# mousecpn/Boosting-R-CNN

Measured on AMD Instinct MI355X. Metric: images/sec (1333x800) Boosting R-CNN R50-PAFPN inference, higher is better.
Workload: dtype f32; 1 GPU; boosting_rcnn_r50_pafpn_1x_utdac.py inference (model(return_loss=False, rescale=True): device pass + result copy + bbox2result), batch 8 x 3x800x1344 per GPU, f32 MFMA conv stack, 1000 pre-NMS / 256 proposals per image, seeded synthetic weights; global_batch=8, parallelism=dp1

## Files before the change

### boosting-r-cnn_amd/csrc/nms.hip

```cpp
#include <cstdlib>
#include "common.h"
#include <cstring>
#include <rocprim/rocprim.hpp>

namespace {

__global__ void iota_kernel(int32_t* __restrict__ v, int32_t* __restrict__ v2, int64_t n) {
    int64_t i = (int64_t)blockIdx.x * blockDim.x + threadIdx.x;
    if (i < n) { v[i] = (int32_t)i; v2[i] = (int32_t)i; }
}

__global__ void gather_boxes_kernel(const float* __restrict__ boxes,
                                    const int32_t* __restrict__ sorted_idx,
                                    float* __restrict__ sboxes, float* __restrict__ sareas,
                                    int64_t n, int offset) {
    int64_t i = (int64_t)blockIdx.x * blockDim.x + threadIdx.x;
    if (i >= n) return;
    const float4 b = *reinterpret_cast<const float4*>(boxes + (size_t)sorted_idx[i] * 4);
    *reinterpret_cast<float4*>(sboxes + (size_t)i * 4) = b;
    sareas[i] = (b.z - b.x + offset) * (b.w - b.y + offset);
}

__global__ __launch_bounds__(64) void nms_mask_kernel(const float* __restrict__ sboxes,
                                                      const float* __restrict__ sareas,
                                                      const int32_t* __restrict__ seg_begin,
                                                      const int32_t* __restrict__ seg_end,
                                                      unsigned long long* __restrict__ mask,
                                                      int words, float thr, int offset) {
    const int col_t = blockIdx.x, row_t = blockIdx.y, seg = blockIdx.z;
    if (col_t < row_t) return;
    const int beg = seg_begin[seg], len = seg_end[seg] - beg;
    if (row_t * 64 >= len || col_t * 64 >= len) return;
    __shared__ float4 cb[64];
    __shared__ float ca[64];
    const int lane = threadIdx.x;
    const int cj = col_t * 64 + lane;
    if (cj < len) {
        cb[lane] = *reinterpret_cast<const float4*>(sboxes + (size_t)(beg + cj) * 4);
        ca[lane] = sareas[beg + cj];
    }
    __syncthreads();
    const int ri = row_t * 64 + lane;
    if (ri >= len) return;
    const float4 a = *reinterpret_cast<const float4*>(sboxes + (size_t)(beg + ri) * 4);
    const float aarea = sareas[beg + ri];
    const int ncol = min(64, len - col_t * 64);
    unsigned long long bits = 0ull;
    const int jstart = (row_t == col_t) ? lane + 1 : 0;
    for (int j = jstart; j < ncol; j++) {
        const float4 b = cb[j];
        const float xx1 = fmaxf(a.x, b.x), yy1 = fmaxf(a.y, b.y);
        const float xx2 = fminf(a.z, b.z), yy2 = fminf(a.w, b.w);
        const float w = fmaxf(0.f, xx2 - xx1 + offset), h = fmaxf(0.f, yy2 - yy1 + offset);
        const float inter = w * h;
        const float ovr = inter / (aarea + ca[j] - inter);
        if (ovr > thr) bits |= 1ull << j;
    }
    mask[(size_t)(beg + ri) * words + col_t] = bits;
}

__global__ __launch_bounds__(256) void nms_reduce_kernel(const unsigned long long* __restrict__ mask,
                                                         const int32_t* __restrict__ sorted_idx,
                                                         const int32_t* __restrict__ seg_begin,
                                                         const int32_t* __restrict__ seg_end,
                                                         int64_t* __restrict__ keep,
                                                         int32_t* __restrict__ num_keep, int words,
                                                         int max_keep) {
    extern __shared__ unsigned long long remv[];
    __shared__ int sh_count;
    const int seg = blockIdx.x, tid = threadIdx.x, lane = tid & 63, wave = tid >> 6;
    const int beg = seg_begin[seg], len = seg_end[seg] - beg;
    const int nchunk = (len + 63) >> 6;
    unsigned long long* kept_sh = remv + words;
    for (int w = tid; w < nchunk; w += 256) remv[w] = 0ull;
    if (tid == 0) sh_count = 0;
    __syncthreads();
    int count = 0;
    unsigned long long diag_next = 0ull, diag_cur = 0ull;
    if (wave == 0 && lane < len) diag_next = mask[(size_t)(beg + lane) * words];
    {
        unsigned nlo, nhi;
        asm volatile("v_mov_b32 %0, %2\n\tv_mov_b32 %1, %3"
                     : "=v"(nlo), "=v"(nhi)
                     : "v"((unsigned)diag_next), "v"((unsigned)(diag_next >> 32)));
        diag_cur = ((unsigned long long)nhi << 32) | nlo;
    }
    for (int c = 0; c < nchunk; c++) {
        const unsigned long long* mchunk = mask + (size_t)(beg + c * 64) * words;
        const int w0 = c + 1 + lane;
        unsigned long long pre[16];
#pragma unroll
        for (int j = 0; j < 16; j++) {
            const int r = wave * 16 + j;
            pre[j] = (w0 < nchunk && c * 64 + r < len) ? mchunk[(size_t)r * words + w0] : 0ull;
// ... 211 lines not shown
    if (k < num[b]) {
        const long long src = keep[(size_t)b * T + k];
        const float4 bx = *reinterpret_cast<const float4*>(c_boxes + src * 4);
        d[0] = bx.x; d[1] = bx.y; d[2] = bx.z; d[3] = bx.w; d[4] = c_scores[src];
        ids_kept[i] = c_ids[src];
    } else {
        d[0] = d[1] = d[2] = d[3] = d[4] = 0.f;
        ids_kept[i] = -1;
    }
}


__device__ __forceinline__ unsigned order_key(float f) {
    const unsigned u = __float_as_uint(f);
    return (u & 0x80000000u) ? ~u : (u | 0x80000000u);
}

template <int THREADS>
__global__ __launch_bounds__(THREADS) void seg_sort_gather_kernel(const float* __restrict__ boxes,
                                                              const float* __restrict__ scores,
                                                              const int32_t* __restrict__ seg_begin,
                                                              const int32_t* __restrict__ seg_end,
                                                              int32_t* __restrict__ idx_out, float* __restrict__ sboxes,
                                                              float* __restrict__ sareas, int offset) {
    extern __shared__ unsigned long long comp[];
    const int seg = blockIdx.x, tid = threadIdx.x;
    const int beg = seg_begin[seg], len = seg_end[seg] - beg;
    if (len <= 0) return;
    int P = 64;
    while (P < len) P <<= 1;
    for (int i = tid; i < P; i += THREADS)
        comp[i] = i < len ? (((unsigned long long)(~order_key(scores[beg + i])) << 32) | (unsigned)i) : ~0ull;
    __syncthreads();
    for (int k = 2; k <= P; k <<= 1) {
        for (int j = k >> 1; j > 0; j >>= 1) {
            for (int t = tid; t < (P >> 1); t += THREADS) {
                const int lo = ((t & ~(j - 1)) << 1) | (t & (j - 1));
                const int hi = lo | j;
                const unsigned long long a = comp[lo], b = comp[hi];
                const bool up = (lo & k) == 0;
                if ((a > b) == up) { comp[lo] = b; comp[hi] = a; }
            }
            __syncthreads();
        }
    }
    for (int i = tid; i < len; i += THREADS) {
        const int src = beg + (int)(comp[i] & 0xffffffffu);
        idx_out[beg + i] = src;
        const float4 b = *reinterpret_cast<const float4*>(boxes + (size_t)src * 4);
        *reinterpret_cast<float4*>(sboxes + (size_t)(beg + i) * 4) = b;
        sareas[beg + i] = (b.z - b.x + offset) * (b.w - b.y + offset);
    }
}

__global__ __launch_bounds__(1024) void nms_collect_sorted_kernel(const long long* __restrict__ keep,
                                                                 const int* __restrict__ num, const int* __restrict__ ranges,
                                                                 const float* __restrict__ c_boxes,
                                                                 const float* __restrict__ c_scores,
                                                                 const long long* __restrict__ c_ids,
                                                                 const float* __restrict__ new_scores,
                                                                 float* __restrict__ dets, long long* __restrict__ ids_kept,
                                                                 int* __restrict__ n_kept, int T, int L, int K) {
    extern __shared__ unsigned long long comp[];
    __shared__ int s_off[BRCNN_MAX_LEVELS + 1];
    const int b = blockIdx.x, tid = threadIdx.x;
    if (tid == 0) {
        int o = 0;
        for (int l = 0; l < L; l++) { s_off[l] = o; o += num[b * L + l]; }
        s_off[L] = o;
    }
    __syncthreads();
    const int cnt = s_off[L];
    int P = 64;
    while (P < cnt) P <<= 1;
    for (int l = 0; l < L; l++) {
        const int beg = ranges[2 * (b * L + l)], n_l = s_off[l + 1] - s_off[l];
        for (int i = tid; i < n_l; i += 1024) {
            const long long src = keep[beg + i];
            const float sc = new_scores ? new_scores[(size_t)(beg + i) * 5 + 4] : c_scores[src];
            comp[s_off[l] + i] = ((unsigned long long)(~order_key(sc)) << 32) | (unsigned)(src - (long long)b * T);
        }
    }
    for (int i = cnt + tid; i < P; i += 1024) comp[i] = ~0ull;
    __syncthreads();
    for (int k = 2; k <= P; k <<= 1) {
        for (int j = k >> 1; j > 0; j >>= 1) {
            for (int t = tid; t < (P >> 1); t += 1024) {
                const int lo = ((t & ~(j - 1)) << 1) | (t & (j - 1));
                const int hi = lo | j;
                const unsigned long long a = comp[lo], c = comp[hi];
                const bool up = (lo & k) == 0;
                if ((a > c) == up) { comp[lo] = c; comp[hi] = a; }
            }
            __syncthreads();
        }
    }
    const int kept = cnt < K ? cnt : K;
    if (tid == 0) n_kept[b] = kept;
    for (int k = tid; k < K; k += 1024) {
        float* d = dets + ((size_t)b * K + k) * 5;
        if (k < kept) {
            const unsigned long long c = comp[k];
            const size_t src = (size_t)b * T + (unsigned)(c & 0xffffffffu);
            const float4 bx = *reinterpret_cast<const float4*>(c_boxes + src * 4);
            const unsigned key = ~(unsigned)(c >> 32);
            const unsigned u = (key & 0x80000000u) ? (key & 0x7fffffffu) : ~key;
            d[0] = bx.x; d[1] = bx.y; d[2] = bx.z; d[3] = bx.w; d[4] = __uint_as_float(u);
            if (ids_kept) ids_kept[(size_t)b * K + k] = c_ids[src];
        } else {
            d[0] = d[1] = d[2] = d[3] = d[4] = 0.f;
            if (ids_kept) ids_kept[(size_t)b * K + k] = -1;
        }
    }
}

}

static int g_nms_lds_sort = getenv("BRCNN_NMS_RADIX") ? 0 : 1;

BRCNN_API size_t brcnn_nms_workspace_bytes(int64_t n, int num_segments, int64_t max_segment_len) {
    if (n <= 0 || num_segments <= 0) return 256;
    if (max_segment_len <= 0 || max_segment_len > n) max_segment_len = n;
    const int words = (int)((max_segment_len + 63) / 64);
    return carve(nullptr, n, num_segments, words).total;
}

BRCNN_API int brcnn_nms(const float* boxes, const float* scores, const int32_t* seg_begin,
                        const int32_t* seg_end, int num_segments, int64_t n, int64_t max_segment_len, float iou_threshold,
                        int offset, int max_keep, int64_t* keep, int32_t* num_keep, void* workspace,
                        size_t workspace_bytes, void* stream) {
    if (n < 0 || num_segments <= 0 || (offset != 0 && offset != 1) || !seg_begin || !seg_end || !num_keep)
        return BRCNN_EINVAL;
    hipStream_t s = (hipStream_t)stream;
    if (n == 0) {
        BRCNN_HIP_CHECK(hipMemsetAsync(num_keep, 0, sizeof(int32_t) * num_segments, s));
        return 0;
    }
    if (!boxes || !scores || !keep || !workspace || max_segment_len <= 0 || max_segment_len > n)
        return BRCNN_EINVAL;
    if (n > 0x7fffffffLL) return BRCNN_EINVAL;
    const int words = (int)((max_segment_len + 63) / 64);
    NmsWs w = carve(workspace, n, num_segments, words);
    if (w.total > workspace_bytes) return BRCNN_EINVAL;

    if (max_segment_len <= 16384 && g_nms_lds_sort) {
        int P = 64;
        while (P < max_segment_len) P <<= 1;
        static bool attr_done = false;
        if (!attr_done) {
            BRCNN_HIP_CHECK(hipFuncSetAttribute((const void*)seg_sort_gather_kernel<1024>,
                                                hipFuncAttributeMaxDynamicSharedMemorySize, 16384 * 8));
            attr_done = true;
        }
        if (max_segment_len <= 512)
            hipLaunchKernelGGL(seg_sort_gather_kernel<256>, dim3(num_segments), dim3(256), (size_t)P * 8, s, boxes, scores,
                               seg_begin, seg_end, w.idx_out, w.sboxes, w.sareas, offset);
        else
            hipLaunchKernelGGL(seg_sort_gather_kernel<1024>, dim3(num_segments), dim3(1024), (size_t)P * 8, s, boxes, scores,
                               seg_begin, seg_end, w.idx_out, w.sboxes, w.sareas, offset);
        BRCNN_LAUNCH_CHECK();
    } else {
        hipLaunchKernelGGL(iota_kernel, dim3(brcnn_cdiv(n, 256)), dim3(256), 0, s, w.idx_in, w.idx_out, n);
        BRCNN_LAUNCH_CHECK();
        size_t tmp = w.sort_tmp_bytes;
        BRCNN_HIP_CHECK((rocprim::segmented_radix_sort_pairs_desc(
            w.sort_tmp, tmp, scores, w.keys_out, (const int32_t*)w.idx_in, w.idx_out, (unsigned)n,
            (unsigned)num_segments, seg_begin, seg_end, 0, 32, s, false)));
        hipLaunchKernelGGL(gather_boxes_kernel, dim3(brcnn_cdiv(n, 256)), dim3(256), 0, s, boxes,
                           (const int32_t*)w.idx_out, w.sboxes, w.sareas, n, offset);
        BRCNN_LAUNCH_CHECK();
    }
    hipLaunchKernelGGL(nms_mask_kernel, dim3(words, words, num_segments), dim3(64), 0, s,
                       (const float*)w.sboxes, (const float*)w.sareas, seg_begin, seg_end, w.mask, words,
                       iou_threshold, offset);
    BRCNN_LAUNCH_CHECK();
    hipLaunchKernelGGL(nms_reduce_kernel, dim3(num_segments), dim3(256), (size_t)(words + 1) * 8, s,
                       (const unsigned long long*)w.mask, (const int32_t*)w.idx_out, seg_begin, seg_end,
                       keep, num_keep, words, max_keep);
    BRCNN_LAUNCH_CHECK();
    return 0;
}

BRCNN_API int brcnn_nms_prepare(const float* boxes, const float* scores, const int64_t* ids, const uint8_t* valid,
                                float* c_boxes, float* c_scores, int64_t* c_ids, float* nms_boxes, int32_t* ranges,
                                int batch, int slot, void* stream) {
    if (!boxes || !scores || !ids || !valid || !c_boxes || !c_scores || !c_ids || !nms_boxes || !ranges ||
        batch <= 0 || slot <= 0 || (long long)batch * slot >= 0x7fffffffLL)
        return BRCNN_EINVAL;
    LevelBounds lb;
    lb.num = 0;
    hipLaunchKernelGGL(nms_prepare_kernel, dim3(batch), dim3(1024), 0, (hipStream_t)stream, boxes, scores,
                       (const long long*)ids, valid, c_boxes, c_scores, (long long*)c_ids, nms_boxes, ranges, slot, lb);
    BRCNN_LAUNCH_CHECK();
    return 0;
}

BRCNN_API int brcnn_nms_prepare_levels(const float* boxes, const float* scores, const int64_t* ids, const uint8_t* valid,
                                       float* c_boxes, float* c_scores, int64_t* c_ids, float* nms_boxes,
                                       int32_t* ranges, int batch, int slot, int num_levels,
                                       const int* level_sizes_host, void* stream) {
    if (!boxes || !scores || !ids || !valid || !c_boxes || !c_scores || !c_ids || !nms_boxes || !ranges ||
        batch <= 0 || slot <= 0 || (long long)batch * slot >= 0x7fffffffLL || num_levels <= 0 ||
        num_levels > BRCNN_MAX_LEVELS || !level_sizes_host)
// ... 13 lines not shown
    BRCNN_LAUNCH_CHECK();
    return 0;
}

BRCNN_API int brcnn_nms_collect_sorted(const int64_t* keep, const int32_t* num, const int32_t* ranges,
                                       const float* c_boxes, const float* c_scores, const int64_t* c_ids,
                                       const float* new_scores5, float* dets, int64_t* ids_kept, int32_t* n_kept,
                                       int batch, int slot, int num_levels, int max_keep, void* stream) {
    if (!keep || !num || !ranges || !c_boxes || !c_scores || !c_ids || !dets || !n_kept || batch <= 0 || slot <= 0 ||
        slot > 16384 || num_levels <= 0 || num_levels > BRCNN_MAX_LEVELS || max_keep <= 0 || max_keep > slot)
        return BRCNN_EINVAL;
    int P = 64;
    while (P < slot) P <<= 1;
    static bool attr_done = false;
    if (!attr_done) {
        BRCNN_HIP_CHECK(hipFuncSetAttribute((const void*)nms_collect_sorted_kernel,
                                            hipFuncAttributeMaxDynamicSharedMemorySize, 16384 * 8));
        attr_done = true;
    }
    hipLaunchKernelGGL(nms_collect_sorted_kernel, dim3(batch), dim3(1024), (size_t)P * 8, (hipStream_t)stream,
                       (const long long*)keep, num, ranges, c_boxes, c_scores, (const long long*)c_ids, new_scores5, dets,
                       (long long*)ids_kept, n_kept, slot, num_levels, max_keep);
    BRCNN_LAUNCH_CHECK();
    return 0;
}

BRCNN_API int brcnn_nms_collect(const int64_t* keep, const int32_t* num, const float* c_boxes, const float* c_scores,
                                const int64_t* c_ids, float* dets, int64_t* ids_kept, int batch, int slot,
                                int max_keep, void* stream) {
    if (!keep || !num || !c_boxes || !c_scores || !c_ids || !dets || !ids_kept || batch <= 0 || slot <= 0 ||
        max_keep <= 0 || max_keep > slot)
        return BRCNN_EINVAL;
    const int total = batch * max_keep;
    hipLaunchKernelGGL(nms_collect_kernel, dim3((total + 255) / 256), dim3(256), 0, (hipStream_t)stream,
                       (const long long*)keep, num, c_boxes, c_scores, (const long long*)c_ids, dets,
                       (long long*)ids_kept, batch, slot, max_keep);
    BRCNN_LAUNCH_CHECK();
    return 0;
}
```

### boosting-r-cnn_amd/csrc/policy.h

```cpp
#pragma once

namespace brcnn {

struct Policy {
    int use_dma = 1;
    int force_wm = 0, force_nt = 0;
    int no_fast = 0;
    int pp_f32_n128 = 1;
    int pp_f32_mode = 1;
    int f32_tile_sk = 1;
    int f32_tile_sk_per_cu = 0;
    int f32_winograd = 1;
    int f32_winograd_chunks = 1;
    int f32_winograd_layer = 1;
    int f32_winograd_gemm = 0;
    int f32_winograd_sk = 1;
    int f32_winograd_sk_per_cu = 0;
    int f32_winograd_sk_wgs = 0;
    int f32_winograd_ring = 0;
    int f32_winograd_tower_gemm = 0;

    int dcn_fused = 1;

    int bf16_tile = 0;
// ... 4 lines not shown
    int pp128_mode = 1;
    int pp128_min_k = 4096;
    int pp128_max_t88 = 128;
    int sk_spin_limit = 1 << 24;
    int sk_drop_publish = 0;
    int stream_mode = 1;

    int wgrad_bf16_tile = 0;
    int wgrad_slabs = 1;
    int wgrad_slot_pct = 75;
    int wgrad_slot_pct_big = 75;
    int wgrad_two_pass = 24;
    int wgrad_pp_mode = 1;
    int wgrad_pp_slot_pct = 75;
    int wgrad_pp_two_pass = 24;
    int wgrad_pp_fuse = 0;

    int roi_exact = 0;
    int roi_stream_c = 3;
    int roi_prep = 0;
    int roi_rpw = 0;
    int roi_order = 1;
    int roi_gather_chunks = -1;
};
extern Policy g_policy;

struct Counters {
    int f32_tile_sk_launches = 0;
    int f32_tile_sk_wgs = 0;
    int wgrad_pp_launches = 0;
    int pp_f32_launches = 0;
    int pp_f32_rows = 0;
    int pp_f32_cols = 0;
    int pp_bf16_launches = 0;
    int pp128_bf16_launches = 0;
    int stream1x1_launches = 0;
    int sk_chain_fills = 0;
    int sk_par_fills = 0;
    int sk_last_wgs = 0;
    int bf16_tile_launches = 0;
    int bf16_tile_rows = 0;
    int bf16_tile_cols = 0;
    int bf16_tile_waves = 0;
    int bf16_tile_stages = 0;
    int wgrad_bf16_tile_launches = 0;
    int wgrad_bf16_last_tile = 0;
    int f32_winograd_launches = 0;
    int f32_winograd_tiles = 0;
    int f32_winograd_layer_launches = 0;
    int f32_winograd_layer_variant = 0;
    int f32_winograd_sk_launches = 0;
    int f32_winograd_sk_last_wgs = 0;
    int f32_winograd_tower_variant = 0;
    int f32_winograd_last_ring = 0;
    int dcn_fused_launches = 0;
    int dcn_im2col_launches = 0;
    int roi_ordered_launches = 0;
    int roi_prepared_launches = 0;
    int roi_gather_chunked = 0;
    int roi_gather_last_ch = 0;
};
extern Counters g_counters;
inline void count(int& c) { c = (c + 1) & 0x7fffffff; }

int wino_layer_rule(int tiles, int cin, int cout);
int wino_gemm_rule(int tiles, int cout);
int wino_gemm_variant(int tiles, int cout);
int wino_persistent_rule(int workgroup_tiles, int units, int cus, int per_cu);
int wino_tower_gemm_rule(int tiles, int cout);
int wino_ring_rule(int workgroup_tiles, int cin);

}
```

### boosting-r-cnn_amd/csrc/policy.hip

```cpp
#include "common.h"
#include "policy.h"

__attribute__((require_constant_initialization)) brcnn::Policy brcnn::g_policy;
__attribute__((require_constant_initialization)) brcnn::Counters brcnn::g_counters;
using brcnn::g_counters, brcnn::g_policy;

BRCNN_API int brcnn_conv_set_tile(int wm, int nt) {
    if (wm == -1) { g_policy.use_dma = nt; return 0; }
    if (wm == -3) { if (nt < 0 || nt > 2) return BRCNN_EINVAL; g_policy.pp_f32_n128 = nt; return 0; }
    if (wm == -4) { if (nt != 0 && nt != 1) return BRCNN_EINVAL; g_policy.no_fast = nt; return 0; }
    if (wm == -5) { if (nt < 0 || nt > 2) return BRCNN_EINVAL; g_policy.f32_tile_sk = nt; return 0; }
    if (wm == -7) { if (nt < 0 || nt > 8) return BRCNN_EINVAL; g_policy.f32_tile_sk_per_cu = nt; return 0; }
    if (wm == -6) return nt == 0 ? g_counters.f32_tile_sk_launches : nt == 1 ? g_counters.f32_tile_sk_wgs : BRCNN_EINVAL;
    if (wm == -9) {
        int* const c[] = {&g_counters.pp_f32_launches, &g_counters.pp_f32_rows, &g_counters.pp_f32_cols, &g_counters.pp_bf16_launches,
                          &g_counters.pp128_bf16_launches, &g_counters.stream1x1_launches, &g_counters.sk_chain_fills,
                          &g_counters.sk_par_fills, &g_counters.sk_last_wgs, &g_counters.bf16_tile_launches, &g_counters.bf16_tile_rows,
                          &g_counters.bf16_tile_cols, &g_counters.bf16_tile_waves, &g_counters.bf16_tile_stages,
                          &g_counters.wgrad_bf16_tile_launches, &g_counters.wgrad_bf16_last_tile};
        const int count = (int)(sizeof(c) / sizeof(c[0]));
        if (nt < -1 || nt >= count) return BRCNN_EINVAL;
        if (nt == -1) {
            for (int* q : c) *q = 0;
            g_counters.f32_winograd_launches = g_counters.f32_winograd_tiles = 0;
            g_counters.dcn_fused_launches = g_counters.dcn_im2col_launches = 0;
            g_counters.f32_winograd_layer_launches = g_counters.f32_winograd_layer_variant = 0;
            g_counters.f32_winograd_sk_launches = g_counters.f32_winograd_sk_last_wgs = g_counters.f32_winograd_tower_variant = 0;
            g_counters.f32_winograd_last_ring = 0;
            return 0;
        }
        const int n = *c[nt];
        *c[nt] = 0;
        return n;
    }
    if (wm == -11) {
        if (nt == 0 || nt == 1) { g_policy.f32_winograd = nt; return 0; }
        if (nt == 2) return g_policy.f32_winograd;
        if (nt >= 11 && nt <= 18) { g_policy.f32_winograd_chunks = nt - 10; return 0; }
        return BRCNN_EINVAL;
    }
    if (wm == -12) {
        if (nt != 0 && nt != 1) return BRCNN_EINVAL;
        int& c = nt == 0 ? g_counters.f32_winograd_launches : g_counters.f32_winograd_tiles;
        const int n = c;
        c = 0;
        return n;
    }
    if (wm == -13) {
        if (nt >= 0 && nt <= 2) { g_policy.dcn_fused = nt; return 0; }
        if (nt == 3) return g_policy.dcn_fused;
        if (nt != 10 && nt != 11) return BRCNN_EINVAL;
// ... 7 lines not shown
        if (nt == 3) return g_policy.f32_winograd_layer;
        if (nt >= 20 && nt <= 23) { g_policy.f32_winograd_gemm = nt - 20; return 0; }
        if (nt == 24) return g_policy.f32_winograd_gemm;
        if (nt != 10 && nt != 11) return BRCNN_EINVAL;
        int& c = nt == 10 ? g_counters.f32_winograd_layer_launches : g_counters.f32_winograd_layer_variant;
        const int n = c;
        c = 0;
        return n;
    }
    if (wm == -16) {
        if (nt >= 0 && nt <= 2) { g_policy.f32_winograd_sk = nt; return 0; }
        if (nt == 3) return g_policy.f32_winograd_sk;
        if (nt == 20 || nt == 21 || nt == 23) { g_policy.f32_winograd_tower_gemm = nt - 20; return 0; }
        if (nt == 24) return g_policy.f32_winograd_tower_gemm;
        if (nt >= 30 && nt <= 38) { g_policy.f32_winograd_sk_per_cu = nt - 30; return 0; }
        if (nt == 39) return g_policy.f32_winograd_sk_per_cu;
        if (nt == 40 || nt == 42 || nt == 43) { g_policy.f32_winograd_ring = nt - 40; return 0; }
        if (nt == 49) return g_policy.f32_winograd_ring;
        if (nt >= 1000 && nt <= 1000 + 2048) { g_policy.f32_winograd_sk_wgs = nt - 1000; return 0; }
        if (nt == 999) return g_policy.f32_winograd_sk_wgs;
        if (nt < 10 || nt > 13) return BRCNN_EINVAL;
        int& c = nt == 10 ? g_counters.f32_winograd_sk_launches : nt == 11 ? g_counters.f32_winograd_sk_last_wgs
                 : nt == 12 ? g_counters.f32_winograd_tower_variant : g_counters.f32_winograd_last_ring;
        const int n = c;
        c = 0;
        return n;
    }
    if (wm == -2) { if (nt != 0 && nt != 1 && nt != 2 && nt != 128 && nt != 256) return BRCNN_EINVAL; g_policy.pp_f32_mode = nt; return 0; }
    if ((wm != 0 && wm != 1 && wm != 2 && wm != 4) || nt < 0 || nt > 2) return BRCNN_EINVAL;
    g_policy.force_wm = wm;
    g_policy.force_nt = nt;
    return 0;
}

int brcnn::wino_gemm_rule(int tiles, int cout) {
    (void)tiles; (void)cout;
    return 3;
}

int brcnn::wino_layer_rule(int tiles, int cin, int cout) {
    if (cin != cout) return 0;
    if (cin == 256) return tiles >= 5250;
    if (cin == 512) return tiles >= 444;
    return 0;
}

// ... 136 lines not shown
```

### boosting-r-cnn_amd/dense_heads.py

```python
import copy

import torch
import torch.distributed as dist
import torch.nn as nn

from . import ops
from .blocks import (ConvModule, PackedCache, Scale, bias_init_with_prob, pack_weight, to_nhwc)
from .postprocess import batched_nms_images
from .core import (anchor_inside_flags, bbox_overlaps, const_rows, images_to_levels, multi_apply, unmap)
from .registry import (HEADS, build_anchor_generator, build_assigner, build_bbox_coder,
                       build_loss, build_sampler)

EPS = 1e-12


def cat_rows(feats):
    from .autograd import cat_rows as _cr
    return _cr(list(feats))


def _nchw_rows(lst):
    return torch.cat([t.permute(0, 2, 3, 1).reshape(-1, t.shape[1]) for t in lst], 0).float()


# ... 302 lines not shown
                for b in range(B):
                    p1, v1 = ops.rpn_decode(topk_inds[b:b + 1], reg_nhwc[lvl][b:b + 1],
                                            self._base_anchors(lvl, device), (h, w), stride,
                                            self.bbox_coder.means, self.bbox_coder.stds,
                                            img_metas[b]['img_shape'][:2], cfg.min_bbox_size,
                                            pred_scale=rs)
                    pl.append(p1)
                    vl.append(v1)
                props, valid = torch.cat(pl), torch.cat(vl)
            if cfg.min_bbox_size < 0:
                valid = torch.ones_like(valid)
            sc_l.append(score)
            pr_l.append(props)
            va_l.append(valid.bool())
            id_l.append(torch.full((B, score.shape[1]), lvl, dtype=torch.long, device=device))
        scores = torch.cat(sc_l, 1)
        props = torch.cat(pr_l, 1)
        valid = torch.cat(va_l, 1)
        ids = torch.cat(id_l, 1)
        return self._proposals_from_candidates(props, scores, ids, valid, sc_l, nms_cfg, cfg)

    @staticmethod
    def _proposals_from_candidates(props, scores, ids, valid, sc_l, nms_cfg, cfg):
        if scores.shape[1] >= nms_cfg.get('split_thr', 10000):
            from .postprocess import batched_nms_images_by_level
            return batched_nms_images_by_level(props, scores, ids, valid, [s_.shape[1] for s_ in sc_l],
                                               nms_cfg['iou_threshold'], cfg.max_per_img,
                                               nms_cfg.get('offset', 0))
        dets, _, num = batched_nms_images(props, scores, ids, valid, nms_cfg['iou_threshold'],
                                          cfg.max_per_img, nms_cfg.get('offset', 0))
        return dets, num


@HEADS.register_module()
class ATSSRPNHead(AnchorHead):
    def __init__(self, in_channels, num_classes=1, stacked_convs=4, conv_cfg=None, gamma=1,
                 atss=False, bridge=False, last_conv='norm', aug_reg_loss=None,
                 norm_cfg=dict(type='GN', num_groups=32, requires_grad=True),
                 loss_centerness=dict(type='CrossEntropyLoss', use_sigmoid=True, loss_weight=0.5),
                 init_cfg=None, num_convs=1, **kwargs):
        assert not atss, 'atss=True (ATSSAssigner targets) is outside the shipped boosting configs'
        assert not bridge and last_conv == 'norm', 'bridge / dcn / aspp variants are out of scope'
        self.stacked_convs, self.conv_cfg, self.norm_cfg = stacked_convs, conv_cfg, norm_cfg
        self.last_conv = last_conv
        super().__init__(num_classes, in_channels, init_cfg=init_cfg, **kwargs)
        self.loss_centerness = build_loss(loss_centerness)
        self.gamma, self.atss, self.bridge = gamma, atss, bridge
# ... 2154 lines not shown
```

### boosting-r-cnn_amd/lib.py

```python
import ctypes
import os

_HERE = os.path.dirname(os.path.abspath(__file__))
LIB_PATH = os.environ.get('BRCNN_LIB_PATH') or os.path.join(_HERE, 'lib', 'libbrcnn_hip.so')
_lib = None

c_int, c_i64, c_f32, c_f64, c_ptr, c_size = (ctypes.c_int, ctypes.c_int64, ctypes.c_float,
                                             ctypes.c_double, ctypes.c_void_p, ctypes.c_size_t)

SIGNATURES = {
    'brcnn_version': (c_int, []),
    'brcnn_device_count': (c_int, []),
    'brcnn_roi_align_forward': (c_int, [c_ptr] * 5 + [c_int] * 7 + [c_f32] + [c_int] * 4 + [c_ptr]),
    'brcnn_roi_align_backward': (c_int, [c_ptr] * 3 + [c_int] * 7 + [c_f32] + [c_int] * 3 + [c_ptr]),
    'brcnn_roi_extract_forward': (c_int, [c_ptr] * 4 + [c_int] + [c_ptr] * 3 + [c_int] * 6 +
                                  [c_f32, c_int, c_ptr]),
    'brcnn_roi_extract_forward_ordered': (c_int, [c_ptr] * 4 + [c_int] + [c_ptr] * 3 + [c_int] * 6 +
                                          [c_f32, c_int, c_ptr, c_ptr]),
    'brcnn_roi_extract_prep_workspace_bytes': (c_size, [c_int]),
    'brcnn_roi_extract_order_min_rois': (c_int, []),
    'brcnn_roi_extract_forward_prepared': (c_int, [c_ptr] * 4 + [c_int] + [c_ptr] * 3 + [c_int] * 6 +
                                           [c_f32, c_int, c_ptr, c_ptr, c_size, c_ptr]),
    'brcnn_get_tuning': (c_int, [c_ptr]),
    'brcnn_set_tuning': (c_int, [c_ptr]),
    'brcnn_roi_extract_backward': (c_int, [c_ptr] * 4 + [c_int] + [c_ptr] * 2 + [c_int] * 6 +
                                   [c_f32, c_ptr]),
    'brcnn_roi_extract_backward_workspace_bytes': (c_size, [c_int]),
    'brcnn_roi_extract_backward_workspace_bytes_ex': (c_size, [c_int, c_int, c_int, c_int, c_ptr, c_ptr]),
    'brcnn_roi_extract_backward_gather': (c_int, [c_ptr] * 4 + [c_int] + [c_ptr] * 2 + [c_int] * 6 + [c_f32, c_ptr, c_size,
                                                                                                    c_int, c_ptr]),
    'brcnn_roi_extract_backward_gather_add': (c_int, [c_ptr] * 5 + [c_int] + [c_ptr] * 2 + [c_int] * 6 + [c_f32, c_ptr, c_size,
                                                                                                        c_int, c_ptr]),
    'brcnn_nms_workspace_bytes': (c_size, [c_i64, c_int, c_i64]),
    'brcnn_nms': (c_int, [c_ptr] * 4 + [c_int, c_i64, c_i64, c_f32, c_int, c_int, c_ptr, c_ptr,
                                        c_ptr, c_size, c_ptr]),
    'brcnn_softnms_workspace_bytes': (c_size, [c_i64, c_int]),
    'brcnn_softnms': (c_int, [c_ptr] * 4 + [c_int, c_i64, c_f32, c_f32, c_f32, c_int, c_int,
                                            c_ptr, c_ptr, c_ptr, c_ptr, c_size, c_ptr]),
    'brcnn_sigmoid_focal_loss_forward': (c_int, [c_ptr] * 4 + [c_i64, c_i64, c_f32, c_f32, c_ptr]),
    'brcnn_sigmoid_focal_loss_backward': (c_int, [c_ptr] * 4 + [c_i64, c_i64, c_f32, c_f32, c_ptr]),
    'brcnn_conv2d_nhwc': (c_int, [c_ptr] * 6 + [c_int] * 11 + [c_ptr]),
    'brcnn_conv_set_tile': (c_int, [c_int, c_int]),
    'brcnn_clock_probe': (c_int, [c_ptr, c_i64, c_ptr]),
    'brcnn_nms_prepare': (c_int, [c_ptr] * 9 + [c_int, c_int, c_ptr]),
    'brcnn_nms_collect': (c_int, [c_ptr] * 7 + [c_int, c_int, c_int, c_ptr]),
    'brcnn_conv2d_nhwc_scatter2': (c_int, [c_ptr] * 3 + [c_int] * 14 + [c_ptr]),
    'brcnn_conv2d_nhwc_multi': (c_int, [c_ptr] * 6 + [c_int, c_int, c_ptr, c_ptr] + [c_int] * 8 +
                                [c_ptr]),
    'brcnn_winograd_filter_f32': (c_int, [c_ptr, c_ptr] + [c_int] * 5 + [c_ptr]),
    'brcnn_conv3x3_winograd_f32_multi_workspace_bytes': (c_size, [c_int, c_int, c_ptr, c_ptr, c_int]),
    'brcnn_conv3x3_winograd_f32_multi': (c_int, [c_ptr] * 5 + [c_int, c_int, c_ptr, c_ptr, c_int, c_ptr, c_ptr, c_size,
                                                 c_int, c_int, c_ptr, c_ptr] + [c_int] * 7 + [c_ptr]),
    'brcnn_conv3x3_winograd_f32_layer': (c_int, [c_ptr] * 4 + [c_int, c_ptr, c_ptr, c_size] + [c_int] * 10 + [c_ptr]),
    'brcnn_winograd_layer_route': (c_int, [c_int] * 10),
    'brcnn_winograd_layer_gemm_variant': (c_int, [c_int, c_int]),
    'brcnn_winograd_persistent_rule': (c_int, [c_int] * 4),
    'brcnn_groupnorm_nhwc_multi_stats': (c_int, [c_ptr, c_ptr, c_int, c_int, c_ptr, c_int, c_int, c_f32, c_int, c_ptr]),
    'brcnn_conv2d_dgrad_nhwc_multi': (c_int, [c_ptr] * 3 + [c_int, c_int] + [c_ptr] * 4 + [c_int] * 7 +
# ... 284 lines not shown
```

### boosting-r-cnn_amd/ops.py

```python
import math

import numpy as np
import torch
import torch.nn as nn
from torch.autograd import Function
from torch.autograd.function import once_differentiable

from . import lib as _L

LAYOUT_NCHW, LAYOUT_NHWC = 0, 1
DT_F32, DT_BF16, DT_BF16_OUT_F32, DT_F16, DT_F16_OUT_F32 = 0, 1, 2, 3, 4


def _dt(t):
    if t.dtype == torch.float32:
        return DT_F32
    if t.dtype == torch.bfloat16:
        return DT_BF16
    if t.dtype == torch.float16:
        return DT_F16
    raise _L.BrcnnHipError(f'unsupported activation dtype {t.dtype} (fp32, bf16 or fp16)')


def _out_f32(dt):
# ... 154 lines not shown
        order_scratch = k >= _roi_order_min_rois()
    order = torch.empty((k,), dtype=torch.int32, device=rois.device) if order_scratch and k > 0 else None
    nb = int(lib.brcnn_roi_extract_prep_workspace_bytes(k))
    prep = torch.empty(nb, dtype=torch.uint8, device=rois.device) if nb else None
    st = lib.brcnn_roi_extract_forward_prepared(ptrs, hs, ws, sc, L, _ptr(rois), _ptr(out), _ptr(levels), n, c, k, ph, pw,
                                                int(sampling_ratio), float(finest_scale), dt, _ptr(order), _ptr(prep), nb,
                                                _stream())
    _L.check(st, 'brcnn_roi_extract_forward_prepared')
    return out, levels


def nms_segments(boxes, scores, seg_offsets, max_segment_len, iou_threshold, offset=0,
                 max_keep=-1):
    seg_offsets = seg_offsets.contiguous().to(torch.int32)
    ranges = torch.stack([seg_offsets[:-1], seg_offsets[1:]], 1)
    return nms_ranges(boxes, scores, ranges, max_segment_len, iou_threshold, offset, max_keep)


def nms_ranges(boxes, scores, ranges, max_segment_len, iou_threshold, offset=0, max_keep=-1):
    _require_gpu(boxes, scores, ranges)
    boxes = boxes.contiguous().float()
    scores = scores.contiguous().float()
    ranges = ranges.to(torch.int32)
    seg_begin, seg_end = ranges[:, 0].contiguous(), ranges[:, 1].contiguous()
    n = boxes.size(0)
    S = seg_begin.numel()
    keep = torch.empty((max(n, 1),), dtype=torch.int64, device=boxes.device)
    num_keep = torch.zeros((S,), dtype=torch.int32, device=boxes.device)
    if n == 0:
        return keep[:0], num_keep
    lib = _L.load()
    max_segment_len = max(1, min(int(max_segment_len), n))
    wsb = lib.brcnn_nms_workspace_bytes(n, S, max_segment_len)
    ws = _ws(wsb, boxes.device)
    st = lib.brcnn_nms(_ptr(boxes), _ptr(scores), _ptr(seg_begin), _ptr(seg_end), S, n,
                       max_segment_len,
                       float(iou_threshold), int(offset), int(max_keep), _ptr(keep),
                       _ptr(num_keep), _ptr(ws), wsb, _stream())
    _L.check(st, 'brcnn_nms')
    return keep, num_keep


def nms_prepare(boxes, scores, ids, valid, level_sizes=None):
    _require_gpu(boxes, scores, ids, valid)
    B, T = scores.shape
    boxes, scores = boxes.contiguous().float(), scores.contiguous().float()
    ids = ids.contiguous().long()
    valid = valid.contiguous().to(torch.uint8) if valid.dtype != torch.bool else valid.contiguous().view(torch.uint8)
    c_boxes, nms_boxes = torch.empty_like(boxes), torch.empty_like(boxes)
    c_scores, c_ids = torch.empty_like(scores), torch.empty_like(ids)
    if level_sizes is not None:
        import ctypes
        L = len(level_sizes)
        ranges = torch.empty((B * L, 2), dtype=torch.int32, device=boxes.device)
        st = _L.load().brcnn_nms_prepare_levels(_ptr(boxes), _ptr(scores), _ptr(ids), _ptr(valid), _ptr(c_boxes),
                                                _ptr(c_scores), _ptr(c_ids), _ptr(nms_boxes), _ptr(ranges), B, T, L,
                                                (ctypes.c_int * L)(*[int(v) for v in level_sizes]), _stream())
# ... 723 lines not shown
def rpn_topk(scores, k):
    import ctypes
    _require_gpu(*scores)
    L = len(scores)
    B = scores[0].shape[0]
    ns = [int(s.shape[1]) for s in scores]
    for s in scores:
        assert s.dim() == 2 and s.shape[0] == B and s.is_contiguous() and s.dtype == torch.float32
    if not 0 < k <= 4096:
        raise _L.BrcnnHipError(f'rpn_topk: k={k} outside (0, 4096]')
    dev = scores[0].device
    out_s = [torch.empty((B, min(k, n)), dtype=torch.float32, device=dev) for n in ns]
    out_i = [torch.empty((B, min(k, n)), dtype=torch.int64, device=dev) for n in ns]
    pa = lambda ts: (ctypes.c_void_p * L)(*[t.data_ptr() for t in ts])
    lib = _L.load()
    n_arr = (ctypes.c_int * L)(*ns)
    wsb = lib.brcnn_rpn_topk_workspace_bytes(n_arr, L, B, int(k))
    ws = _ws(wsb, dev)
    st = lib.brcnn_rpn_topk(pa(scores), n_arr, L, B, int(k), pa(out_s), pa(out_i), _ptr(ws), wsb, _stream())
    _L.check(st, 'brcnn_rpn_topk')
    return list(zip(out_s, out_i))


def rpn_decode(topk_inds, bbox_pred, base_anchors, feat_hw, stride, means, stds, max_shape,
               min_size, wh_ratio_clip=16 / 1000, pred_scale=1.0):
    import ctypes
    _require_gpu(topk_inds, bbox_pred, base_anchors)
    b, k = topk_inds.shape
    h, w = feat_hw
    a = base_anchors.size(0)
    _, a4, pstride = _last_dim_strided(bbox_pred)
    assert a4 == 4 * a
    props = torch.empty((b, k, 4), dtype=torch.float32, device=bbox_pred.device)
    valid = torch.empty((b, k), dtype=torch.uint8, device=bbox_pred.device)
    m4 = (ctypes.c_float * 4)(*[float(v) for v in means])
    s4 = (ctypes.c_float * 4)(*[float(v) for v in stds])
    sw, sh = (stride, stride) if isinstance(stride, int) else stride
    mh, mw = (float(max_shape[0]), float(max_shape[1])) if max_shape is not None else (0.0, 0.0)
    st = _L.load().brcnn_rpn_decode(_ptr(topk_inds.contiguous()), _ptr(bbox_pred), int(pstride),
                                    float(pred_scale),
                                    _ptr(base_anchors.contiguous().float()), b, k, h, w, a,
                                    int(sw), int(sh), m4, s4, float(wh_ratio_clip), mh, mw,
                                    float(min_size), _ptr(props), _ptr(valid), _stream())
    _L.check(st, 'brcnn_rpn_decode')
    return props, valid

# ... 707 lines not shown
```

### boosting-r-cnn_amd/postprocess.py

```python
import torch

from . import ops

_INDEX_CACHE = {}


def _column_index(cols, device):
    key = (tuple(int(c) for c in cols), str(device))
    t = _INDEX_CACHE.get(key)
    if t is None:
        if len(_INDEX_CACHE) > 256:
            _INDEX_CACHE.clear()
        t = _INDEX_CACHE[key] = torch.tensor(key[0], dtype=torch.long, device=device)
    return t


def batched_nms_images(boxes, scores, ids, valid, iou_threshold, max_keep, offset=0, fused=None):
    B, T = scores.shape
    device = scores.device
    K = max_keep if max_keep > 0 else T
    K = min(K, T)
    if fused is None:
        fused = boxes.is_cuda and boxes.dtype == torch.float32
    if fused:
# ... 32 lines not shown
    return dets, ids_kept, num


def batched_nms_images_by_level(boxes, scores, ids, valid, level_sizes, iou_threshold, max_keep, offset=0,
                                return_ids=False, soft=None, fused=None):
    B, T = scores.shape
    L = len(level_sizes)
    assert sum(level_sizes) == T
    device = scores.device
    K = min(max_keep, T) if max_keep > 0 else T
    if fused is None:
        fused = boxes.is_cuda and boxes.dtype == torch.float32 and T <= 16384 and L <= 8
    if fused:
        c_boxes, c_scores, c_ids, boxes_for_nms, ranges = ops.nms_prepare(boxes, scores, ids, valid,
                                                                          level_sizes=level_sizes)
        sdets = None
        if soft is not None:
            method = {'naive': 0, 'linear': 1, 'gaussian': 2}[soft.get('method', 'linear')]
            sdets, keep, num = ops.soft_nms_ranges(boxes_for_nms.view(-1, 4), c_scores.reshape(-1), ranges,
                                                   iou_threshold, soft.get('sigma', 0.5), soft.get('min_score', 1e-3),
                                                   method, offset)
        else:
            keep, num = ops.nms_ranges(boxes_for_nms.view(-1, 4), c_scores.reshape(-1), ranges, max(level_sizes),
                                       iou_threshold, offset, -1)
        dets, ids_kept, n_kept = ops.nms_collect_sorted(keep, num, ranges, c_boxes, c_scores, c_ids, K, L, sdets)
        if return_ids:
            return dets, ids_kept.to(ids.dtype), n_kept
        return dets, n_kept
    cnt = valid.sum(1)
    dest = torch.cumsum(valid, 1) - 1
    dest = torch.where(valid, dest, torch.full_like(dest, T))

    def compact(x):
        out = torch.zeros((B, T + 1) + tuple(x.shape[2:]), dtype=x.dtype, device=device)
        idx = dest.view(B, T, *([1] * (x.dim() - 2))).expand_as(x)
        out.scatter_(1, idx, x)
        return out[:, :T].contiguous()

    c_boxes, c_scores, c_ids = compact(boxes), compact(scores), compact(ids)
    pos = torch.arange(T, device=device)[None, :]
    in_range = pos < cnt[:, None]
    lowest = torch.finfo(c_boxes.dtype).min
    max_coord = torch.where(in_range[..., None], c_boxes, c_boxes.new_full((), lowest)).amax((1, 2))
    offs = c_ids.to(c_boxes) * (max_coord + 1)[:, None]
    boxes_for_nms = c_boxes + offs[..., None]
    bounds = [0]
    for n in level_sizes:
# ... 36 lines not shown
```

### include/brcnn_hip.h

```cpp
#ifndef BRCNN_HIP_H
#define BRCNN_HIP_H

#include <stddef.h>
#include <stdint.h>

#ifdef __cplusplus
extern "C" {
#endif

#define BRCNN_LAYOUT_NCHW 0
#define BRCNN_LAYOUT_NHWC 1

#define BRCNN_DT_F32 0
#define BRCNN_DT_BF16 1
#define BRCNN_DT_BF16_OUT_F32 2
#define BRCNN_DT_F16 3
#define BRCNN_DT_F16_OUT_F32 4

#define BRCNN_MAX_LEVELS 8
#define BRCNN_MAX_IMAGES 64

int brcnn_version(void);

int brcnn_clock_probe(int64_t *out2, int64_t wall_ticks_100mhz, void *stream);
// ... 79 lines not shown
int brcnn_set_tuning(const brcnn_tuning *t);

int brcnn_nms_prepare(const float *boxes, const float *scores, const int64_t *ids, const uint8_t *valid,
                      float *c_boxes, float *c_scores, int64_t *c_ids, float *nms_boxes, int32_t *ranges,
                      int batch, int slot, void *stream);
int brcnn_nms_collect(const int64_t *keep, const int32_t *num, const float *c_boxes, const float *c_scores,
                      const int64_t *c_ids, float *dets, int64_t *ids_kept, int batch, int slot,
                      int max_keep, void *stream);

int brcnn_nms_prepare_levels(const float *boxes, const float *scores, const int64_t *ids, const uint8_t *valid,
                             float *c_boxes, float *c_scores, int64_t *c_ids, float *nms_boxes,
                             int32_t *ranges, int batch, int slot, int num_levels,
                             const int *level_sizes_host, void *stream);
int brcnn_nms_collect_sorted(const int64_t *keep, const int32_t *num, const int32_t *ranges,
                             const float *c_boxes, const float *c_scores, const int64_t *c_ids,
                             const float *new_scores5, float *dets, int64_t *ids_kept, int32_t *n_kept,
                             int batch, int slot, int num_levels, int max_keep, void *stream);

size_t brcnn_nms_workspace_bytes(int64_t n, int num_segments, int64_t max_segment_len);
int brcnn_nms(const float *boxes, const float *scores, const int32_t *seg_begin,
              const int32_t *seg_end, int num_segments, int64_t n, int64_t max_segment_len, float iou_threshold,
              int offset, int max_keep, int64_t *keep, int32_t *num_keep, void *workspace,
              size_t workspace_bytes, void *stream);

size_t brcnn_softnms_workspace_bytes(int64_t n, int num_segments);
int brcnn_softnms(const float *boxes, const float *scores, const int32_t *seg_begin,
                  const int32_t *seg_end, int num_segments, int64_t n, float iou_threshold, float sigma, float min_score,
                  int method, int offset, float *dets, int64_t *inds, int32_t *num_keep,
                  void *workspace, size_t workspace_bytes, void *stream);

int brcnn_sigmoid_focal_loss_forward(const float *input, const int64_t *target,
                                     const float *weight, float *output, int64_t n, int64_t c,
                                     float gamma, float alpha, void *stream);
int brcnn_sigmoid_focal_loss_backward(const float *input, const int64_t *target,
                                      const float *weight, float *grad_input, int64_t n,
                                      int64_t c, float gamma, float alpha, void *stream);

int brcnn_conv2d_nhwc(const void *x, const void *w, const float *scale, const float *shift,
                      const void *residual, void *y, int batch, int height, int width, int cin,
                      int cout, int kh, int kw, int stride, int pad, int relu, int dtype,
                      void *stream);

int brcnn_conv2d_nhwc_scatter2(const void *x, const void *w, void *y, int batch, int height, int width,
                               int cin, int cout, int kh, int kw, int pad, int out_height,
                               int out_width, int ph, int pw, int origin, int dtype, void *stream);

// ... 552 lines not shown
```

Before: 401.8 images/sec.

## Route RPN proposals through per-level segmented NMS with capped keep count

Enables a policy flag that sends RPN proposal NMS through the per-level batched path even below the split threshold, so each image's levels are suppressed as separate segments. A new strided-ranges NMS entry point reads begin and end offsets directly from the interleaved ranges tensor, which avoids two slicing copies and a zero fill per call. The per-segment keep count is now capped at max_per_img, and the collect kernel is adjusted to count the true total while offsetting by the capped counts. Splitting into smaller segments cuts the quadratic mask work, but per-level suppression is only equivalent to the original batched NMS if boxes from different levels were already kept apart by offsets.

Measured after the change: 403.4 images/sec, median of 5. No clear change (+0.4%).

```diff
diff --git a/boosting-r-cnn_amd/csrc/nms.hip b/boosting-r-cnn_amd/csrc/nms.hip
--- a/boosting-r-cnn_amd/csrc/nms.hip
+++ b/boosting-r-cnn_amd/csrc/nms.hip
@@ -1,5 +1,6 @@
 #include <cstdlib>
 #include "common.h"
+#include "policy.h"
 #include <cstring>
 #include <rocprim/rocprim.hpp>
 
@@ -26,10 +27,10 @@
                                                       const int32_t* __restrict__ seg_begin,
                                                       const int32_t* __restrict__ seg_end,
                                                       unsigned long long* __restrict__ mask,
-                                                      int words, float thr, int offset) {
+                                                      int words, float thr, int offset, int ss) {
     const int col_t = blockIdx.x, row_t = blockIdx.y, seg = blockIdx.z;
     if (col_t < row_t) return;
-    const int beg = seg_begin[seg], len = seg_end[seg] - beg;
+    const int beg = seg_begin[(size_t)seg * ss], len = seg_end[(size_t)seg * ss] - beg;
     if (row_t * 64 >= len || col_t * 64 >= len) return;
     __shared__ float4 cb[64];
     __shared__ float ca[64];
@@ -65,11 +66,11 @@
                                                          const int32_t* __restrict__ seg_end,
                                                          int64_t* __restrict__ keep,
                                                          int32_t* __restrict__ num_keep, int words,
-                                                         int max_keep) {
+                                                         int max_keep, int ss) {
     extern __shared__ unsigned long long remv[];
     __shared__ int sh_count;
     const int seg = blockIdx.x, tid = threadIdx.x, lane = tid & 63, wave = tid >> 6;
-    const int beg = seg_begin[seg], len = seg_end[seg] - beg;
+    const int beg = seg_begin[(size_t)seg * ss], len = seg_end[(size_t)seg * ss] - beg;
     const int nchunk = (len + 63) >> 6;
     unsigned long long* kept_sh = remv + words;
     for (int w = tid; w < nchunk; w += 256) remv[w] = 0ull;
@@ -327,10 +328,10 @@
                                                               const int32_t* __restrict__ seg_begin,
                                                               const int32_t* __restrict__ seg_end,
                                                               int32_t* __restrict__ idx_out, float* __restrict__ sboxes,
-                                                              float* __restrict__ sareas, int offset) {
+                                                              float* __restrict__ sareas, int offset, int ss) {
     extern __shared__ unsigned long long comp[];
     const int seg = blockIdx.x, tid = threadIdx.x;
-    const int beg = seg_begin[seg], len = seg_end[seg] - beg;
+    const int beg = seg_begin[(size_t)seg * ss], len = seg_end[(size_t)seg * ss] - beg;
     if (len <= 0) return;
     int P = 64;
     while (P < len) P <<= 1;
@@ -369,10 +370,17 @@
     extern __shared__ unsigned long long comp[];
     __shared__ int s_off[BRCNN_MAX_LEVELS + 1];
     const int b = blockIdx.x, tid = threadIdx.x;
+    __shared__ int s_total;
     if (tid == 0) {
-        int o = 0;
-        for (int l = 0; l < L; l++) { s_off[l] = o; o += num[b * L + l]; }
+        int o = 0, total = 0;
+        for (int l = 0; l < L; l++) {
+            const int n_l = num[b * L + l];
+            s_off[l] = o;
+            o += new_scores ? n_l : min(n_l, K);
+            total += n_l;
+        }
         s_off[L] = o;
+        s_total = total;
     }
     __syncthreads();
     const int cnt = s_off[L];
@@ -400,7 +408,7 @@
             __syncthreads();
         }
     }
-    const int kept = cnt < K ? cnt : K;
+    const int kept = s_total < K ? s_total : K;
     if (tid == 0) n_kept[b] = kept;
     for (int k = tid; k < K; k += 1024) {
         float* d = dets + ((size_t)b * K + k) * 5;
@@ -430,10 +438,10 @@
     return carve(nullptr, n, num_segments, words).total;
 }
 
-BRCNN_API int brcnn_nms(const float* boxes, const float* scores, const int32_t* seg_begin,
-                        const int32_t* seg_end, int num_segments, int64_t n, int64_t max_segment_len, float iou_threshold,
-                        int offset, int max_keep, int64_t* keep, int32_t* num_keep, void* workspace,
-                        size_t workspace_bytes, void* stream) {
+static int nms_impl(const float* boxes, const float* scores, const int32_t* seg_begin,
+                    const int32_t* seg_end, int ss, int num_segments, int64_t n, int64_t max_segment_len, float iou_threshold,
+                    int offset, int max_keep, int64_t* keep, int32_t* num_keep, void* workspace,
+                    size_t workspace_bytes, void* stream) {
     if (n < 0 || num_segments <= 0 || (offset != 0 && offset != 1) || !seg_begin || !seg_end || !num_keep)
         return BRCNN_EINVAL;
     hipStream_t s = (hipStream_t)stream;
@@ -459,12 +467,13 @@
         }
         if (max_segment_len <= 512)
             hipLaunchKernelGGL(seg_sort_gather_kernel<256>, dim3(num_segments), dim3(256), (size_t)P * 8, s, boxes, scores,
-                               seg_begin, seg_end, w.idx_out, w.sboxes, w.sareas, offset);
+                               seg_begin, seg_end, w.idx_out, w.sboxes, w.sareas, offset, ss);
         else
             hipLaunchKernelGGL(seg_sort_gather_kernel<1024>, dim3(num_segments), dim3(1024), (size_t)P * 8, s, boxes, scores,
-                               seg_begin, seg_end, w.idx_out, w.sboxes, w.sareas, offset);
+                               seg_begin, seg_end, w.idx_out, w.sboxes, w.sareas, offset, ss);
         BRCNN_LAUNCH_CHECK();
     } else {
+        if (ss != 1) return BRCNN_EINVAL;
         hipLaunchKernelGGL(iota_kernel, dim3(brcnn_cdiv(n, 256)), dim3(256), 0, s, w.idx_in, w.idx_out, n);
         BRCNN_LAUNCH_CHECK();
         size_t tmp = w.sort_tmp_bytes;
@@ -477,13 +486,30 @@
     }
     hipLaunchKernelGGL(nms_mask_kernel, dim3(words, words, num_segments), dim3(64), 0, s,
                        (const float*)w.sboxes, (const float*)w.sareas, seg_begin, seg_end, w.mask, words,
-                       iou_threshold, offset);
+                       iou_threshold, offset, ss);
     BRCNN_LAUNCH_CHECK();
     hipLaunchKernelGGL(nms_reduce_kernel, dim3(num_segments), dim3(256), (size_t)(words + 1) * 8, s,
                        (const unsigned long long*)w.mask, (const int32_t*)w.idx_out, seg_begin, seg_end,
-                       keep, num_keep, words, max_keep);
+                       keep, num_keep, words, max_keep, ss);
     BRCNN_LAUNCH_CHECK();
     return 0;
+}
+
+BRCNN_API int brcnn_nms(const float* boxes, const float* scores, const int32_t* seg_begin,
+                        const int32_t* seg_end, int num_segments, int64_t n, int64_t max_segment_len, float iou_threshold,
+                        int offset, int max_keep, int64_t* keep, int32_t* num_keep, void* workspace,
+                        size_t workspace_bytes, void* stream) {
+    return nms_impl(boxes, scores, seg_begin, seg_end, 1, num_segments, n, max_segment_len, iou_threshold, offset, max_keep,
+                    keep, num_keep, workspace, workspace_bytes, stream);
+}
+
+BRCNN_API int brcnn_nms_ranges(const float* boxes, const float* scores, const int32_t* ranges, int num_segments, int64_t n,
+                               int64_t max_segment_len, float iou_threshold, int offset, int max_keep, int64_t* keep,
+                               int32_t* num_keep, void* workspace, size_t workspace_bytes, void* stream) {
+    if (!ranges || max_segment_len > 16384) return BRCNN_EINVAL;
+    brcnn::count(brcnn::g_counters.nms_ranges_calls);
+    return nms_impl(boxes, scores, ranges, ranges + 1, 2, num_segments, n, max_segment_len, iou_threshold, offset, max_keep,
+                    keep, num_keep, workspace, workspace_bytes, stream);
 }
 
 BRCNN_API int brcnn_nms_prepare(const float* boxes, const float* scores, const int64_t* ids, const uint8_t* valid,
@@ -543,6 +569,7 @@
                        (const long long*)keep, num, ranges, c_boxes, c_scores, (const long long*)c_ids, new_scores5, dets,
                        (long long*)ids_kept, n_kept, slot, num_levels, max_keep);
     BRCNN_LAUNCH_CHECK();
+    brcnn::count(brcnn::g_counters.nms_collect_sorted_launches);
     return 0;
 }
 
diff --git a/boosting-r-cnn_amd/csrc/policy.h b/boosting-r-cnn_amd/csrc/policy.h
--- a/boosting-r-cnn_amd/csrc/policy.h
+++ b/boosting-r-cnn_amd/csrc/policy.h
@@ -50,6 +50,8 @@
     int roi_rpw = 0;
     int roi_order = 1;
     int roi_gather_chunks = -1;
+
+    int rpn_nms_by_level = 1;
 };
 extern Policy g_policy;
 
@@ -87,6 +89,8 @@
     int roi_prepared_launches = 0;
     int roi_gather_chunked = 0;
     int roi_gather_last_ch = 0;
+    int nms_collect_sorted_launches = 0;
+    int nms_ranges_calls = 0;
 };
 extern Counters g_counters;
 inline void count(int& c) { c = (c + 1) & 0x7fffffff; }
diff --git a/boosting-r-cnn_amd/csrc/policy.hip b/boosting-r-cnn_amd/csrc/policy.hip
--- a/boosting-r-cnn_amd/csrc/policy.hip
+++ b/boosting-r-cnn_amd/csrc/policy.hip
@@ -27,6 +27,7 @@
             g_counters.f32_winograd_layer_launches = g_counters.f32_winograd_layer_variant = 0;
             g_counters.f32_winograd_sk_launches = g_counters.f32_winograd_sk_last_wgs = g_counters.f32_winograd_tower_variant = 0;
             g_counters.f32_winograd_last_ring = 0;
+            g_counters.nms_collect_sorted_launches = g_counters.nms_ranges_calls = 0;
             return 0;
         }
         const int n = *c[nt];
@@ -80,6 +81,15 @@
         if (nt < 10 || nt > 13) return BRCNN_EINVAL;
         int& c = nt == 10 ? g_counters.f32_winograd_sk_launches : nt == 11 ? g_counters.f32_winograd_sk_last_wgs
                  : nt == 12 ? g_counters.f32_winograd_tower_variant : g_counters.f32_winograd_last_ring;
+        const int n = c;
+        c = 0;
+        return n;
+    }
+    if (wm == -18) {
+        if (nt == 40 || nt == 41) { g_policy.rpn_nms_by_level = nt - 40; return 0; }
+        if (nt == 42) return g_policy.rpn_nms_by_level;
+        if (nt != 20 && nt != 21) return BRCNN_EINVAL;
+        int& c = nt == 20 ? g_counters.nms_collect_sorted_launches : g_counters.nms_ranges_calls;
         const int n = c;
         c = 0;
         return n;
diff --git a/boosting-r-cnn_amd/dense_heads.py b/boosting-r-cnn_amd/dense_heads.py
--- a/boosting-r-cnn_amd/dense_heads.py
+++ b/boosting-r-cnn_amd/dense_heads.py
@@ -348,7 +348,10 @@
 
     @staticmethod
     def _proposals_from_candidates(props, scores, ids, valid, sc_l, nms_cfg, cfg):
-        if scores.shape[1] >= nms_cfg.get('split_thr', 10000):
+        T = scores.shape[1]
+        by_level = props.is_cuda and props.dtype == torch.float32 and T <= 16384 and len(sc_l) <= 8 and \
+            0 < cfg.max_per_img <= T and ops.rpn_nms_by_level_enabled()
+        if T >= nms_cfg.get('split_thr', 10000) or by_level:
             from .postprocess import batched_nms_images_by_level
             return batched_nms_images_by_level(props, scores, ids, valid, [s_.shape[1] for s_ in sc_l],
                                                nms_cfg['iou_threshold'], cfg.max_per_img,
diff --git a/boosting-r-cnn_amd/lib.py b/boosting-r-cnn_amd/lib.py
--- a/boosting-r-cnn_amd/lib.py
+++ b/boosting-r-cnn_amd/lib.py
@@ -34,6 +34,7 @@
     'brcnn_nms_workspace_bytes': (c_size, [c_i64, c_int, c_i64]),
     'brcnn_nms': (c_int, [c_ptr] * 4 + [c_int, c_i64, c_i64, c_f32, c_int, c_int, c_ptr, c_ptr,
                                         c_ptr, c_size, c_ptr]),
+    'brcnn_nms_ranges': (c_int, [c_ptr] * 3 + [c_int, c_i64, c_i64, c_f32, c_int, c_int, c_ptr, c_ptr, c_ptr, c_size, c_ptr]),
     'brcnn_softnms_workspace_bytes': (c_size, [c_i64, c_int]),
     'brcnn_softnms': (c_int, [c_ptr] * 4 + [c_int, c_i64, c_f32, c_f32, c_f32, c_int, c_int,
                                             c_ptr, c_ptr, c_ptr, c_ptr, c_size, c_ptr]),
diff --git a/boosting-r-cnn_amd/ops.py b/boosting-r-cnn_amd/ops.py
--- a/boosting-r-cnn_amd/ops.py
+++ b/boosting-r-cnn_amd/ops.py
@@ -200,17 +200,22 @@
     boxes = boxes.contiguous().float()
     scores = scores.contiguous().float()
     ranges = ranges.to(torch.int32)
-    seg_begin, seg_end = ranges[:, 0].contiguous(), ranges[:, 1].contiguous()
     n = boxes.size(0)
-    S = seg_begin.numel()
+    S = ranges.shape[0]
     keep = torch.empty((max(n, 1),), dtype=torch.int64, device=boxes.device)
-    num_keep = torch.zeros((S,), dtype=torch.int32, device=boxes.device)
     if n == 0:
-        return keep[:0], num_keep
+        return keep[:0], torch.zeros((S,), dtype=torch.int32, device=boxes.device)
+    num_keep = torch.empty((S,), dtype=torch.int32, device=boxes.device)
     lib = _L.load()
     max_segment_len = max(1, min(int(max_segment_len), n))
     wsb = lib.brcnn_nms_workspace_bytes(n, S, max_segment_len)
     ws = _ws(wsb, boxes.device)
+    if ranges.is_contiguous() and max_segment_len <= 16384:
+        st = lib.brcnn_nms_ranges(_ptr(boxes), _ptr(scores), _ptr(ranges), S, n, max_segment_len, float(iou_threshold),
+                                  int(offset), int(max_keep), _ptr(keep), _ptr(num_keep), _ptr(ws), wsb, _stream())
+        _L.check(st, 'brcnn_nms_ranges')
+        return keep, num_keep
+    seg_begin, seg_end = ranges[:, 0].contiguous(), ranges[:, 1].contiguous()
     st = lib.brcnn_nms(_ptr(boxes), _ptr(scores), _ptr(seg_begin), _ptr(seg_end), S, n,
                        max_segment_len,
                        float(iou_threshold), int(offset), int(max_keep), _ptr(keep),
@@ -980,6 +985,10 @@
     return list(zip(out_s, out_i))
 
 
+def rpn_nms_by_level_enabled():
+    return _L.load().brcnn_conv_set_tile(-18, 42) == 1
+
+
 def rpn_decode(topk_inds, bbox_pred, base_anchors, feat_hw, stride, means, stds, max_shape,
                min_size, wh_ratio_clip=16 / 1000, pred_scale=1.0):
     import ctypes
diff --git a/boosting-r-cnn_amd/postprocess.py b/boosting-r-cnn_amd/postprocess.py
--- a/boosting-r-cnn_amd/postprocess.py
+++ b/boosting-r-cnn_amd/postprocess.py
@@ -78,7 +78,7 @@
                                                    method, offset)
         else:
             keep, num = ops.nms_ranges(boxes_for_nms.view(-1, 4), c_scores.reshape(-1), ranges, max(level_sizes),
-                                       iou_threshold, offset, -1)
+                                       iou_threshold, offset, K)
         dets, ids_kept, n_kept = ops.nms_collect_sorted(keep, num, ranges, c_boxes, c_scores, c_ids, K, L, sdets)
         if return_ids:
             return dets, ids_kept.to(ids.dtype), n_kept
diff --git a/include/brcnn_hip.h b/include/brcnn_hip.h
--- a/include/brcnn_hip.h
+++ b/include/brcnn_hip.h
@@ -125,6 +125,9 @@
               const int32_t *seg_end, int num_segments, int64_t n, int64_t max_segment_len, float iou_threshold,
               int offset, int max_keep, int64_t *keep, int32_t *num_keep, void *workspace,
               size_t workspace_bytes, void *stream);
+int brcnn_nms_ranges(const float *boxes, const float *scores, const int32_t *ranges, int num_segments, int64_t n,
+                     int64_t max_segment_len, float iou_threshold, int offset, int max_keep, int64_t *keep,
+                     int32_t *num_keep, void *workspace, size_t workspace_bytes, void *stream);
 
 size_t brcnn_softnms_workspace_bytes(int64_t n, int num_segments);
 int brcnn_softnms(const float *boxes, const float *scores, const int32_t *seg_begin,
```
